# skhu101/TDNN-F_NAS

Measured on AMD Instinct MI355X. Metric: LF-MMI training frames/sec per node (SWBD 7q TDNN-F), higher is better.
Workload: dtype f32

## Files before the change

tdnn-f_nas_amd/csrc/abi_tdnn.hip:

```cpp
#include <dlfcn.h>
#include <stdlib.h>
#include <string.h>

#include <string>

#include "common.h"
#include "gemm_f32.h"
#include "planes_gemm.h"

namespace tdnnf {

static thread_local std::string g_last_error;

void set_error(const char *fmt, ...) {
  char buf[1024];
  va_list ap;
  va_start(ap, fmt);
  vsnprintf(buf, sizeof(buf), fmt, ap);
  va_end(ap);
  g_last_error = buf;
}
int hip_status(hipError_t e, const char *what) {
  set_error("HIP error %d (%s) in %s", (int)e, hipGetErrorString(e), what);
  return TDNNF_EHIP;
// ... 4 lines not shown
  return o;
}

namespace {
typedef int (*roctx_push_t)(const char *);
typedef int (*roctx_pop_t)();
roctx_push_t g_roctx_push = nullptr;
roctx_pop_t g_roctx_pop = nullptr;
bool roctx_ready() {
  static const bool ok = [] {
    const char *e = getenv("TDNNF_ROCTX");
    if (e && atoi(e) == 0) return false;
    for (const char *lib : {"librocprofiler-sdk-roctx.so", "librocprofiler-sdk-roctx.so.1", "libroctx64.so", "libroctx64.so.4"}) {
      void *h = dlopen(lib, RTLD_NOW | RTLD_GLOBAL);
      if (!h) continue;
      g_roctx_push = (roctx_push_t)dlsym(h, "roctxRangePushA");
      g_roctx_pop = (roctx_pop_t)dlsym(h, "roctxRangePop");
      if (g_roctx_push && g_roctx_pop) return true;
    }
    return false;
  }();
  return ok;
}
}
TraceRange::TraceRange(const char *name) : on(roctx_ready()) {
  if (on) g_roctx_push(name);
}
TraceRange::~TraceRange() {
  if (on) g_roctx_pop();
}

static bool tdnn_rows_ok(const tdnnf_tdnn_indexes *ix, int rows_in, int N) {
  if (!ix || ix->num_offsets < 1 || ix->num_offsets > TDNNF_MAX_OFFSETS || ix->row_stride < 1) return false;
  for (int i = 0; i < ix->num_offsets; i++) {
    const long long need = (long long)ix->row_offsets[i] + (long long)ix->row_stride * N - (ix->row_stride - 1);
    if (ix->row_offsets[i] < 0 || (N > 0 && rows_in < need)) return false;
  }
  return true;
}

}

using namespace tdnnf;

extern "C" {

const char *tdnnf_last_error(void) { return g_last_error.c_str(); }
int tdnnf_abi_version(void) { return 1; }

static int *option_slot(const char *name) {
  Options &o = options();
  if (!name) return nullptr;
  const struct { const char *n; int *p; } table[] = {{"ng_grouped", &o.ng_grouped}, {"ng_fuse", &o.ng_fuse}, {"ng_early_in", &o.ng_early_in},
                                                     {"wgrad_stream", &o.wgrad_stream}, {"gemm_ring", &o.gemm_ring}, {"planes", &o.planes}, {"den_split", &o.den_split}, {"phase_events", &o.phase_events}, {"wgrad_lag", &o.wgrad_lag}, {"ng_bk", &o.ng_bk}, {"ng_valu", &o.ng_valu}, {"ng_pform", &o.ng_pform}, {"planes_group", &o.planes_group}, {"xent_behind_den", &o.xent_behind_den}, {"ng_early_fork", &o.ng_early_fork}, {"ng_diag_skip", &o.ng_diag_skip}, {"wgrad_small", &o.wgrad_small}, {"splitk_per_cu", &o.splitk_per_cu}, {"gemm_alt_taps", &o.gemm_alt_taps}, {"reverse_passes", &o.reverse_passes}, {"splitk_partial_round", &o.splitk_partial_round}, {"wgrad_on_caller", &o.wgrad_on_caller}, {"den_mw_test_abort", &o.den_mw_test_abort}, {"planes_check_bound", &o.planes_check_bound}, {"den_gamma_pairs", &o.den_gamma_pairs}};
  for (auto &e : table)
    if (strcmp(e.n, name) == 0) return e.p;
  return nullptr;
}
int tdnnf_set_option(const char *name, int value) {
  int *p = option_slot(name);
  TDNNF_REQUIRE(p, "set_option: unknown option '%s' (ng_grouped, ng_fuse, ng_early_in, wgrad_stream, gemm_ring, planes, den_split)", name ? name : "(null)");
  *p = value;
  return TDNNF_OK;
}
int tdnnf_get_option(const char *name, int *value) {
  int *p = option_slot(name);
  TDNNF_REQUIRE(p && value, "get_option: unknown option '%s'", name ? name : "(null)");
  *value = *p;
  return TDNNF_OK;
}

}

namespace tdnnf {
int tdnn_propagate_impl(const tdnnf_tdnn_indexes *ix, const tdnnf_mat *in, const float *W, int ldw, int Do, int Di,
                        const float *bias, const float *eff_coef, int init_mode, int relu, tdnnf_mat *out, tdnnf_stream stream,
                        float *colstats, int *colstats_rows) {
  TDNNF_REQUIRE(mat_ok(in) && mat_ok(out) && W, "tdnn_propagate: bad matrices");
  TDNNF_REQUIRE(Do > 0 && Di > 0 && in->cols == Di && out->cols == Do, "tdnn_propagate: dims: in.cols=%d Di=%d out.cols=%d Do=%d",
                in ? in->cols : -1, Di, out ? out->cols : -1, Do);
  TDNNF_REQUIRE(tdnn_rows_ok(ix, in->rows, out->rows), "tdnn_propagate: input has too few rows for the time offsets");
  TDNNF_REQUIRE(ldw >= ix->num_offsets * Di, "tdnn_propagate: ldw < K*Di");
  TDNNF_REQUIRE(init_mode >= 0 && init_mode <= 2 && (init_mode != 1 || bias), "tdnn_propagate: init_mode 1 needs a bias");
  RowsGemmArgs a;
  memset(&a, 0, sizeof(a));
  a.A = in->data;
  a.lda = (long long)in->stride * ix->row_stride;
  a.B = W;
  a.ldb = ldw;
  a.C = out->data;
  a.ldc = out->stride;
  a.M = out->rows;
  a.N = Do;
  a.bias = bias;
  a.coef = eff_coef;
  a.init_mode = init_mode;
  a.relu = relu;
  a.colstats = colstats;
  a.colstats_rows = colstats_rows;
  a.nseg = ix->num_offsets;
  for (int i = 0; i < a.nseg; i++) {
    a.seg[i].a_off = (long long)ix->row_offsets[i] * in->stride;
    a.seg[i].b_off = (long long)i * Di;
    a.seg[i].klen = Di;
    a.seg[i].m_lo = 0;
    a.seg[i].m_hi = out->rows;
  }
// ... 201 lines not shown
```

tdnn-f_nas_amd/csrc/chain.hip:

```cpp
#include <math.h>
#include <string.h>

#include <algorithm>

#include <vector>

#include "common.h"
#include "gemm_f32.h"

struct tdnnf_den_graph {
  int H, A, P;
  struct Sell {
    int nrows, nslices;
    int *base;
    unsigned *row;
    uint2 *arc;
    uint4 *arc4;
    long long entries;
    int mw_max_arcs[9];
  } by_dst, by_src, by_pdf;
  float *init;
  float init_sum;
};

struct tdnnf_supervision {
  int B, T;
  int num_states, num_arcs;
  float weight;
  int *seq_state_begin;
  int *state_time;
  float *final_logprob;
  int *in_begin, *in_src, *in_pdf;
  float *in_lp;
  int *out_begin, *out_dst, *out_pdf;
  float *out_lp;
  int *frame_state_begin;
  int max_states_per_seq;
};

namespace tdnnf {
namespace {

constexpr int kDenThreads = 1024;
typedef float f32x4 __attribute__((ext_vector_type(4)));

__device__ __forceinline__ float block_sum(float v, float *red, int nwaves) {
  for (int o = 32; o > 0; o >>= 1) v += __shfl_xor(v, o, 64);
  __syncthreads();
  if ((threadIdx.x & 63) == 0) red[threadIdx.x >> 6] = v;
  __syncthreads();
  float s = 0.f;
  for (int w = 0; w < nwaves; w++) s += red[w];
  return s;
}

__device__ __forceinline__ float exp_limited(float v) {
  v = v < -30.f ? -30.f : (v > 30.f ? 30.f : v);
  return expf(v);
}

struct DenDev {
  int H, P;
  tdnnf_den_graph::Sell by_dst, by_src, by_pdf;
  const float *init;
  float init_sum;
};

constexpr int kDenRowRegs = 8;
struct RowAhead {
  float v[kDenRowRegs];
  __device__ __forceinline__ void load(const float *yr, int P, int tid) {
#pragma unroll
    for (int i = 0; i < kDenRowRegs; i++) {
      const int p = tid + i * kDenThreads;
      v[i] = p < P ? yr[p] : 0.f;
    }
  }
};

template <class Term>
__device__ __forceinline__ float sell_row_sum(const uint2 *ap, int w, Term term) {
  float acc = 0.f;
  int j = 0;
  for (; j + 8 <= w; j += 8) {
    uint2 a[8];
#pragma unroll
    for (int u = 0; u < 8; u++) a[u] = ap[(j + u) * 64];
#pragma unroll
    for (int u = 0; u < 8; u++) acc += term(a[u]);
  }
  if (j + 4 <= w) {
    uint2 a[4];
#pragma unroll
    for (int u = 0; u < 4; u++) a[u] = ap[(j + u) * 64];
#pragma unroll
    for (int u = 0; u < 4; u++) acc += term(a[u]);
    j += 4;
  }
  if (j < w) {
    uint2 a[3];
#pragma unroll
    for (int u = 0; u < 3; u++) a[u] = ap[min(j + u, w - 1) * 64];
#pragma unroll
    for (int u = 0; u < 3; u++) acc += (j + u < w) ? term(a[u]) : 0.f;
  }
  return acc;
}

constexpr int kDenFastSlots = 4, kDenFastStates = 4;
template <bool LDS_STATE, bool FAST = false>
__global__ __launch_bounds__(kDenThreads) void den_forward_kernel(DenDev g, MatView y, int B, int T, float leaky,
                                                                  float *alpha_all, float *asum_all, int Hs,
                                                                  double *logprob, float *gstate, const unsigned *only_if, int res_cap) {
  extern __shared__ __attribute__((aligned(16))) float smem[];
  __shared__ float red[kDenThreads / 64];
  if (only_if && *only_if == 0) return;
  const int s = blockIdx.x, tid = threadIdx.x;
  const int H = g.H, P = g.P;
  float *x = smem;
  float *prev = LDS_STATE ? smem + ((P + 3) & ~3) : gstate + (size_t)s * 2 * Hs;
  float *nxt = smem + ((P + 3) & ~3) + Hs;
  uint2 *lres = reinterpret_cast<uint2 *>(smem + ((P + 3) & ~3) + (LDS_STATE ? Hs : 0) + (FAST ? Hs : 0));
  for (int i = tid; i < res_cap; i += kDenThreads) lres[i] = g.by_dst.arc[i];
  int sb0[kDenFastSlots], sw[kDenFastSlots];
  unsigned srow[kDenFastSlots];
  float hinit[kDenFastStates];
// ... 589 lines not shown
  constexpr int kRows = 8;
  const int nslot = g.by_pdf.nslices * 64, ln = tid & 63;
  auto pa = [&](const uint2 a, int f) {
#pragma clang fp contract(off)
    return __uint_as_float(a.y) * smem[f * L + (a.x & 0xffffu)];
  };
  auto pb = [&](const uint2 a, int f) { return smem[f * L + H4 + (a.x >> 16)]; };
  for (int s0 = tid; s0 < nslot; s0 += kRows * kGamma2Threads) {
    int b0[kRows], w[kRows];
    unsigned row[kRows];
#pragma unroll
    for (int k = 0; k < kRows; k++) {
      const int slot = s0 + k * kGamma2Threads;
      b0[k] = 0;
      w[k] = 0;
      row[k] = 0xffffffffu;
      if (slot < nslot) {
        b0[k] = g.by_pdf.base[slot >> 6];
        w[k] = (g.by_pdf.base[(slot >> 6) + 1] - b0[k]) >> 6;
        row[k] = g.by_pdf.row[slot];
      }
    }
#pragma unroll
    for (int k = 0; k < kRows; k++) {
      if (row[k] == 0xffffffffu) continue;
      float acc[2];
      sell_row_sums<2>(g.by_pdf.arc + b0[k] + ln, w[k], acc, pa, pb);
#pragma unroll
      for (int f = 0; f < 2; f++) smem[f * L + 2 * H4 + row[k]] = scale[f] * acc[f];
    }
  }
  __syncthreads();
  constexpr int kOut = 6;
  for (int p0 = tid; p0 < P; p0 += kOut * kGamma2Threads) {
    float yv[2][kOut];
#pragma unroll
    for (int f = 0; f < 2; f++)
#pragma unroll
      for (int i = 0; i < kOut; i++) {
        const int p = p0 + i * kGamma2Threads;
        yv[f][i] = f < nf && p < P ? y.data[(size_t)((t0 + f) * B + s) * y.stride + p] : 0.f;
      }
#pragma unroll
    for (int f = 0; f < 2; f++) {
      if (f >= nf) break;
      const float *o = smem + f * L + 2 * H4;
      float *dr = deriv.data + (size_t)((t0 + f) * B + s) * deriv.stride;
#pragma unroll
      for (int i = 0; i < kOut; i++) {
        const int p = p0 + i * kGamma2Threads;
        if (p < P) dr[p] = o[p] * exp_limited(yv[f][i]);
      }
    }
  }
}
constexpr int kWideBatch = 8;
constexpr int kWideSlices = 2;

struct WideDims {
  int B, NG, SG;
};

typedef unsigned uv4 __attribute__((ext_vector_type(4)));

__global__ __launch_bounds__(256) void den_wide_prep_kernel(MatView y, WideDims d, int P, float *xT) {
  __shared__ float tile[64][65];
  const int t = blockIdx.z, p0 = blockIdx.x * 64, s0 = blockIdx.y * 64, tx = threadIdx.x & 63, ty = threadIdx.x >> 6;
  for (int i = ty; i < 64; i += 4) {
    const int sq = s0 + i, p = p0 + tx;
    tile[i][tx] = (sq < d.B && p < P) ? exp_limited(y.data[(size_t)(t * d.B + sq) * y.stride + p]) : 0.f;
  }
  __syncthreads();
  for (int i = ty; i < 64; i += 4) {
    const int p = p0 + i, sq = s0 + tx;
    if (p < P && sq < d.NG * d.SG) xT[(((size_t)t * d.NG + sq / d.SG) * P + p) * d.SG + sq % d.SG] = tile[tx][i];
  }
}
__global__ __launch_bounds__(256) void den_wide_unprep_kernel(const float *dT, WideDims d, int P, MatView deriv) {
  __shared__ float tile[64][65];
  const int t = blockIdx.z, p0 = blockIdx.x * 64, s0 = blockIdx.y * 64, tx = threadIdx.x & 63, ty = threadIdx.x >> 6;
  for (int i = ty; i < 64; i += 4) {
    const int p = p0 + i, sq = s0 + tx;
    tile[i][tx] = (p < P && sq < d.B) ? dT[(((size_t)t * d.NG + sq / d.SG) * P + p) * d.SG + sq % d.SG] : 0.f;
  }
  __syncthreads();
  for (int i = ty; i < 64; i += 4) {
    const int sq = s0 + i, p = p0 + tx;
    if (sq < d.B && p < P) deriv.data[(size_t)(t * d.B + sq) * deriv.stride + p] = tile[tx][i];
  }
}

__global__ __launch_bounds__(256) void den_wide_init_kernel(DenDev g, WideDims d, int Hs, bool ones, float *v, float *norm) {
  const long long total = (long long)d.NG * Hs * d.SG;
  for (long long e = blockIdx.x * 256LL + threadIdx.x; e < total; e += gridDim.x * 256LL) {
    const int h = (int)((e / d.SG) % Hs);
    v[e] = h < g.H ? (ones ? 1.0f : g.init[h]) : 0.f;
  }
  for (long long e = blockIdx.x * 256LL + threadIdx.x; e < d.B; e += gridDim.x * 256LL) norm[e] = g.init_sum;
}

template <int SG>
struct WideLane {
  static constexpr int RL = 64 / SG;
  static constexpr int IT = 16 / RL;
  int grp, blk, sl, rl, sq, wave, lane;
  bool on;
// ... 811 lines not shown
    TDNNF_HIP(hipStreamWaitEvent(aux, ev_fork, 0));
    int G = mw_groups(g, B, T);
    MwDev *md = mw_dev();
    if (!md) G = 0;
    if (G > 0 && !md->fallbacks) {
      if (hipHostMalloc((void **)&md->fallbacks, sizeof(unsigned), hipHostMallocMapped) != hipSuccess) {
        (void)hipGetLastError();
        md->fallbacks = nullptr;
        G = 0;
      } else {
        *md->fallbacks = 0;
      }
    }
    if (G > 0 && *(volatile unsigned *)md->fallbacks != 0) {
      fprintf(stderr, "tdnnf: the multi-workgroup denominator recursion timed out (its workgroups were not co-resident); the one-workgroup kernels redid the "
                      "minibatch and are used from here on (this device)\n");
      md->off = true;
      G = 0;
    }
    const size_t stage_b = G > 0 ? 256 * (size_t)((std::max(g->by_dst.nslices, g->by_src.nslices) + G - 1) / G) : 0;
    const size_t lds_f = G > 0 ? sizeof(float) * (P4 + H4) + 8 * (size_t)g->by_dst.mw_max_arcs[G] + stage_b : 0;
    const size_t lds_b = G > 0 ? sizeof(float) * (P4 + H4) + 8 * (size_t)g->by_src.mw_max_arcs[G] + stage_b : 0;
    if (G > 0) {
      TDNNF_HIP(hipFuncSetAttribute((const void *)den_mw_kernel<0>, hipFuncAttributeMaxDynamicSharedMemorySize, (int)lds_f));
      TDNNF_HIP(hipFuncSetAttribute((const void *)den_mw_kernel<1>, hipFuncAttributeMaxDynamicSharedMemorySize, (int)lds_b));
      int occ_f = 0, occ_b = 0;
      if (hipOccupancyMaxActiveBlocksPerMultiprocessor(&occ_f, den_mw_kernel<0>, kDenThreads, lds_f) != hipSuccess ||
          hipOccupancyMaxActiveBlocksPerMultiprocessor(&occ_b, den_mw_kernel<1>, kDenThreads, lds_b) != hipSuccess || occ_f < 1 || occ_b < 1 ||
          md->cus <= 0 || 2 * B * G > md->cus) {
        (void)hipGetLastError();
        G = 0;
      }
    }
    if (G > 0) {
      float *mw = S_all + (size_t)B * (T + 1) + 32;
      MwCtl ctl;
      ctl.NSp = (int)mw_slots(g);
      ctl.ctr = reinterpret_cast<unsigned long long *>((reinterpret_cast<uintptr_t>(mw) + 15) & ~(uintptr_t)15);
      ctl.abort_flag = reinterpret_cast<unsigned *>(ctl.ctr + 2 * B);
      ctl.xf = reinterpret_cast<float *>(ctl.ctr + 2 * B + 2);
      ctl.xb = ctl.xf + (size_t)B * 2 * ctl.NSp;
      TDNNF_HIP(hipMemsetAsync(ctl.ctr, 0, sizeof(unsigned long long) * (2 * B + 2), s));
      if (options().den_mw_test_abort) TDNNF_HIP(hipMemsetAsync(ctl.abort_flag, 1, 1, s));
      TDNNF_HIP(hipEventRecord(ev_fork, s));
      TDNNF_HIP(hipStreamWaitEvent(aux, ev_fork, 0));
      hipLaunchKernelGGL(den_mw_kernel<0>, dim3(B * G), dim3(kDenThreads), lds_f, s, gd, ctl, G, yv, B, T, leaky, b.alpha, b.asum, b.p.Hs, b.den_lp);
      hipLaunchKernelGGL(den_mw_kernel<1>, dim3(B * G), dim3(kDenThreads), lds_b, aux, gd, ctl, G, yv, B, T, leaky, b_all, S_all, b.p.Hs, (double *)nullptr);
      hipLaunchKernelGGL(den_forward_kernel<true>, dim3(B), dim3(kDenThreads), b.p.lds_fwd, s, gd, yv, B, T, leaky, b.alpha, b.asum, b.p.Hs, b.den_lp, b.gstate,
                         (const unsigned *)ctl.abort_flag, 0);
      hipLaunchKernelGGL(den_beta_kernel<false>, dim3(B), dim3(kDenThreads), lds_beta, aux, gd, yv, B, T, leaky, b_all, S_all, b.p.Hs, (const unsigned *)ctl.abort_flag, 0);
      hipLaunchKernelGGL(den_mw_check_kernel, dim3(1), dim3(64), 0, s, (const unsigned *)ctl.abort_flag, md->fallbacks);
    } else {
      const bool fast = g->by_dst.nslices * 64 <= kDenFastSlots * kDenThreads && g->by_src.nslices * 64 <= kDenFastSlots * kDenThreads && g->H <= kDenFastStates * kDenThreads;
      const size_t lf = b.p.lds_fwd + (fast ? sizeof(float) * b.p.Hs : 0), lb = lds_beta + (fast ? sizeof(float) * H4 : 0);
      int res_f = 0, res_b = 0;
      if (md && md->cus > 0 && 2 * B >= md->cus) {
        const size_t budget = 150 * 1024;
        if (lf < budget) res_f = (int)std::min<long long>(g->by_dst.entries, (long long)((budget - lf) / 8)) & ~63;
        if (lb < budget) res_b = (int)std::min<long long>(g->by_src.entries, (long long)((budget - lb) / 8)) & ~63;
      }
      (void)hipGetLastError();
      const size_t lds_f2 = lf + 8 * (size_t)res_f, lds_b2 = lb + 8 * (size_t)res_b;
      if (fast) {
        TDNNF_HIP(hipFuncSetAttribute((const void *)den_forward_kernel<true, true>, hipFuncAttributeMaxDynamicSharedMemorySize, (int)lds_f2));
        TDNNF_HIP(hipFuncSetAttribute((const void *)den_beta_kernel<true>, hipFuncAttributeMaxDynamicSharedMemorySize, (int)lds_b2));
        hipLaunchKernelGGL((den_forward_kernel<true, true>), dim3(B), dim3(kDenThreads), lds_f2, s, gd, yv, B, T, leaky, b.alpha, b.asum, b.p.Hs, b.den_lp, b.gstate,
                           (const unsigned *)nullptr, res_f);
        hipLaunchKernelGGL(den_beta_kernel<true>, dim3(B), dim3(kDenThreads), lds_b2, aux, gd, yv, B, T, leaky, b_all, S_all, b.p.Hs, (const unsigned *)nullptr, res_b);
      } else {
        TDNNF_HIP(hipFuncSetAttribute((const void *)den_forward_kernel<true>, hipFuncAttributeMaxDynamicSharedMemorySize, (int)lds_f2));
        TDNNF_HIP(hipFuncSetAttribute((const void *)den_beta_kernel<false>, hipFuncAttributeMaxDynamicSharedMemorySize, (int)lds_b2));
        hipLaunchKernelGGL(den_forward_kernel<true>, dim3(B), dim3(kDenThreads), lds_f2, s, gd, yv, B, T, leaky, b.alpha, b.asum, b.p.Hs, b.den_lp, b.gstate,
                           (const unsigned *)nullptr, res_f);
        hipLaunchKernelGGL(den_beta_kernel<false>, dim3(B), dim3(kDenThreads), lds_b2, aux, gd, yv, B, T, leaky, b_all, S_all, b.p.Hs, (const unsigned *)nullptr, res_b);
      }
    }
    TDNNF_HIP(hipEventRecord(ev_join, aux));
    TDNNF_HIP(hipStreamWaitEvent(s, ev_join, 0));
    if (ev_recursions) {
      TDNNF_HIP(hipEventRecord(ev_recursions, s));
      if (ev_recorded) *ev_recorded = true;
    }
    if (options().den_gamma_pairs != 1 && 2 * lds_gamma + sizeof(float) * kGamma2Threads / 64 <= kLdsBytes) {
      TDNNF_HIP(hipFuncSetAttribute((const void *)den_gamma2_kernel, hipFuncAttributeMaxDynamicSharedMemorySize, (int)(2 * lds_gamma)));
      hipLaunchKernelGGL(den_gamma2_kernel, dim3((T + 1) / 2, B), dim3(kGamma2Threads), 2 * lds_gamma, s, gd, yv, B, T, leaky, b.alpha, b_all, S_all, b.p.Hs, -sp->weight, dv);
    } else {
      TDNNF_HIP(hipFuncSetAttribute((const void *)den_gamma_kernel, hipFuncAttributeMaxDynamicSharedMemorySize, (int)lds_gamma));
      hipLaunchKernelGGL(den_gamma_kernel, dim3(T, B), dim3(kGammaThreads), lds_gamma, s, gd, yv, B, T, leaky, b.alpha, b_all, S_all, b.p.Hs, -sp->weight, dv);
    }
  } else if (b.p.lds_state) {
    TDNNF_HIP(hipFuncSetAttribute((const void *)den_backward_kernel<true>, hipFuncAttributeMaxDynamicSharedMemorySize, (int)b.p.lds_bwd));
    if (g->by_dst.nslices * 64 <= kDenFastSlots * kDenThreads && g->H <= kDenFastStates * kDenThreads) {
      const size_t lf = b.p.lds_fwd + sizeof(float) * b.p.Hs;
      TDNNF_HIP(hipFuncSetAttribute((const void *)den_forward_kernel<true, true>, hipFuncAttributeMaxDynamicSharedMemorySize, (int)lf));
      hipLaunchKernelGGL((den_forward_kernel<true, true>), dim3(B), dim3(kDenThreads), lf, s, gd, yv, B, T, leaky, b.alpha, b.asum, b.p.Hs, b.den_lp, b.gstate, (const unsigned *)nullptr, 0);
    } else {
      TDNNF_HIP(hipFuncSetAttribute((const void *)den_forward_kernel<true>, hipFuncAttributeMaxDynamicSharedMemorySize, (int)b.p.lds_fwd));
      hipLaunchKernelGGL(den_forward_kernel<true>, dim3(B), dim3(kDenThreads), b.p.lds_fwd, s, gd, yv, B, T, leaky, b.alpha, b.asum, b.p.Hs, b.den_lp, b.gstate, (const unsigned *)nullptr, 0);
    }
    hipLaunchKernelGGL(den_backward_kernel<true>, dim3(B), dim3(kDenThreads), b.p.lds_bwd, s, gd, yv, B, T, leaky, b.alpha, b.asum, b.p.Hs, -sp->weight, dv, b.gstate);
  } else {
    hipLaunchKernelGGL(den_forward_kernel<false>, dim3(B), dim3(kDenThreads), b.p.lds_fwd, s, gd, yv, B, T, leaky, b.alpha, b.asum, b.p.Hs, b.den_lp, b.gstate, (const unsigned *)nullptr, 0);
    hipLaunchKernelGGL(den_backward_kernel<false>, dim3(B), dim3(kDenThreads), b.p.lds_bwd, s, gd, yv, B, T, leaky, b.alpha, b.asum, b.p.Hs, -sp->weight, dv, b.gstate);
  }
  TDNNF_LAUNCH_CHECK();
  return TDNNF_OK;
}
float chain_supervision_weight(const tdnnf_supervision *sp) { return sp->weight; }
int chain_num_recursion(const tdnnf_supervision *sp, const tdnnf_den_graph *g, const tdnnf_mat *y, void *ws, hipStream_t s) {
  const int B = sp->B, T = sp->T;
  ChainBufs b = chain_bufs(g, B, T, ws);
  const MatView none{nullptr, 0, 0, 0};
  hipLaunchKernelGGL(numerator_kernel, dim3(B), dim3(64), 0, s, sup_dev(sp), view(y), none, b.la, b.lb, b.num_lp, b.xent, none, none, 0.f, 1);
  TDNNF_LAUNCH_CHECK();
  return TDNNF_OK;
}
// ... 65 lines not shown
```

tdnn-f_nas_amd/csrc/common.h:

```cpp
#pragma once
#include <hip/hip_runtime.h>
#include <stdarg.h>
#include <stdio.h>

#include "tdnnf_hip.h"

namespace tdnnf {

struct MatView {
  float *data;
  int rows, cols, stride;
};
inline MatView view(const tdnnf_mat *m) { return MatView{m->data, m->rows, m->cols, m->stride}; }

void set_error(const char *fmt, ...);
int hip_status(hipError_t e, const char *what);

inline bool mat_ok(const tdnnf_mat *m) {
  return m && m->rows >= 0 && m->cols >= 0 && m->stride >= m->cols && (m->data || m->rows * m->cols == 0);
}
inline bool same_dim(const tdnnf_mat *a, const tdnnf_mat *b) { return a->rows == b->rows && a->cols == b->cols; }

inline bool vec4_ok(const MatView &m) {
  return (reinterpret_cast<uintptr_t>(m.data) & 15) == 0 && m.stride % 4 == 0 && m.cols % 4 == 0;
}

#define TDNNF_REQUIRE(cond, ...)            \
  do {                                      \
    if (!(cond)) {                          \
      ::tdnnf::set_error(__VA_ARGS__);      \
      return TDNNF_EINVAL;                  \
    }                                       \
  } while (0)

#define TDNNF_HIP(expr)                                         \
  do {                                                          \
    hipError_t e__ = (expr);                                    \
    if (e__ != hipSuccess) return ::tdnnf::hip_status(e__, #expr); \
  } while (0)

#define TDNNF_LAUNCH_CHECK(name) TDNNF_HIP(hipGetLastError())

struct Options {
  int ng_grouped = 1;
  int ng_fuse = 1;
  int ng_early_in = 1;
  int wgrad_stream = -1;
  int gemm_ring = 1;
  int planes = 1;
  int den_mw_test_abort = 0;
  int planes_group = 1;
  int planes_check_bound = 0;
  int wgrad_lag = 3;
  int wgrad_on_caller = 0;
  int splitk_partial_round = 1;
  int reverse_passes = 0;
  int gemm_alt_taps = 1;
  int splitk_per_cu = 2;
  int wgrad_small = 0;
  int ng_bk = 0;
  int ng_early_fork = 1;
  int xent_behind_den = -1;
  int ng_pform = 1;
  int ng_valu = 0;
  int ng_diag_skip = 0;
  int phase_events = 0;
  int den_split = -1;
  int den_gamma_pairs = 0;
};
Options &options();

struct TraceRange {
  explicit TraceRange(const char *name);
  ~TraceRange();
  bool on;
};

__host__ __device__ inline float floor_keep_nan(float x, float f) { return x < f ? f : x; }

inline int grid_for(long long work, int block, int cap = 2048) {
  long long g = (work + block - 1) / block;
  if (g > cap) g = cap;
  if (g < 1) g = 1;
  return (int)g;
}

inline unsigned long long tdnnf_decision(unsigned long long step, unsigned long long k) {
  unsigned long long z = step * 0x9E3779B97F4A7C15ULL + k * 0xBF58476D1CE4E5B9ULL + 0x94D049BB133111EBULL;
  z = (z ^ (z >> 30)) * 0xBF58476D1CE4E5B9ULL;
  z = (z ^ (z >> 27)) * 0x94D049BB133111EBULL;
  return (z ^ (z >> 31)) >> 8;
}

constexpr int kFinCols = 8, kFinLanes = 32, kFinThreads = kFinCols * kFinLanes;
inline unsigned finalize_grid(int D) { return (unsigned)((D + kFinCols - 1) / kFinCols); }
#ifdef __HIPCC__
template <int NQ, class Acc>
__device__ __forceinline__ void finalize_sums(const float *partial, int chunks, long long qstride_rows, int D, int nq, Acc (&q)[NQ], Acc *red) {
  const int tc = threadIdx.x & (kFinCols - 1), lane = threadIdx.x / kFinCols, d = blockIdx.x * kFinCols + tc;
#pragma unroll
  for (int k = 0; k < NQ; k++) q[k] = 0;
  if (d < D) {
    const float *p = partial + d;
    const long long qs = qstride_rows * D;
    int c = lane;
    for (; c + 3 * kFinLanes < chunks; c += 4 * kFinLanes) {
      float v[NQ][4];
#pragma unroll
      for (int k = 0; k < NQ; k++) {
        if (k < nq) {
          const float *pk = p + (long long)k * qs;
          v[k][0] = pk[(long long)c * D]; v[k][1] = pk[(long long)(c + kFinLanes) * D];
          v[k][2] = pk[(long long)(c + 2 * kFinLanes) * D]; v[k][3] = pk[(long long)(c + 3 * kFinLanes) * D];
        }
      }
#pragma unroll
      for (int k = 0; k < NQ; k++) {
        if (k < nq) { q[k] += v[k][0]; q[k] += v[k][1]; q[k] += v[k][2]; q[k] += v[k][3]; }
      }
    }
    for (; c < chunks; c += kFinLanes) {
// ... 82 lines not shown
```

tdnn-f_nas_amd/csrc/net.hip:

```cpp
#include <math.h>
#include <string.h>

#include <functional>
#include <string>
#include <vector>

#include "common.h"
#include "fused.h"
#include "gemm_f32.h"
#include "gemm_ring.h"
#include "net.h"
#include "ng.h"
#include "optim_group.h"

namespace tdnnf {
namespace {

struct UpdTable {
  long long begin[129];
  float lr[128];
  float l2coef[128];
};

__global__ void add_scaled_taps_kernel(const float *G, const float *coef, float *acc, int Do, int KDi, int Di) {
// ... 1510 lines not shown
      CK(ng_stats_main(n->ng_in[comp], xin, n->ngc[comp].H_in, n->ngc[comp].part_in, n->ws4, n->ws_bytes, n->s4));
      E.done = n->fb_count;
    }
    if (forked) {
      TDNNF_HIP(hipEventRecord(n->ev_early, n->s4));
      n->early_any = true;
    }
    return TDNNF_OK;
  };
  const bool early_at_fork = n->early_on && !n->wg_on && !n->early_group && options().ng_early_fork != 0;
  if (early_at_fork) {
    CK(finish_refreshes());
    CK(launch_early_in(0));
  }
  const int No = n->Tout * B;
  tdnnf_mat top = M(prev, No, Hd), pl = M(n->prefinal_l_out, No, S);
  if (po_next.base == top.data && po_next.rows == top.rows) po_top = po_next;
  else CK(split(top, 0, kP | kT, &po_top, s, fb_next));
  {
    PlanesHintScope ph(hint_of(po_top), wplanes(n->c_prefinal_l));
    CK(tdnnf_affine_propagate(&top, Wp(n, n->c_prefinal_l), Hd, nullptr, S, &pl, s));
  }
  CK(split(pl, 0, kP | kT, &po_pl, s));
  tdnnf_mat y = M(n->head[0].y, No, P), dy = M(n->d_y, No, P), dx = M(n->d_xent, No, P);
  tdnnf_mat lsm = M(n->xent_logsoftmax, No, P);
  for (int h = 0; h < 2; h++) {
    auto &H = n->head[h];
    tdnnf_mat ar = M(H.aff_relu, No, Hd), lo = M(H.lin_out, No, S), b1 = M(H.bn1_out, No, Hd), b2 = M(H.bn2_out, No, S), yh = M(H.y, No, P);
    FroBound fb_b1;
    {
      PlanesHintScope ph(hint_of(po_pl), wplanes(H.c_affine));
      FroBoundScope fbs(pl_on ? n->fro_buf : nullptr, &fb_b1.blocks);
      CK(affine_relu_bn_stats(n, &ix1, &pl, Wp(n, H.c_affine), S, Hd, S, Bp(n, H.c_affine), nullptr, &ar, H.bn1_memo, H.bn1_stats, s));
    }
    CK(bn_apply_planes(ar, H.bn1_memo, none, 0.f, b1, nullptr, fb_b1, &po_b1[h]));
    if (!po_b1[h].base) CK(split(b1, 0, kP | kT, &po_b1[h], s, fb_b1));
    {
      PlanesHintScope ph(hint_of(po_b1[h]), wplanes(H.c_linear));
      CK(tdnnf_affine_propagate(&b1, Wp(n, H.c_linear), Hd, nullptr, S, &lo, s));
    }
    CK(bn_fwd(n, H.lin_out, H.bn2_out, No, S, H.bn2_memo, H.bn2_stats, s));
    CK(split(b2, 0, kP | kT, &po_b2[h], s));
    {
      PlanesHintScope ph(hint_of(po_b2[h]), wplanes(H.c_output));
      CK(tdnnf_affine_propagate(&b2, Wp(n, H.c_output), S, Bp(n, H.c_output), P, &yh, s));
    }
    if (h == 0) {
      TraceRange trace_den("chain denominator forward-backward (second stream)");
      TDNNF_HIP(hipEventRecord(n->ev_fork, s));
      TDNNF_HIP(hipStreamWaitEvent(n->s2, n->ev_fork, 0));
      const bool den_split = n->den_split;
      TDNNF_HIP(hipStreamWaitEvent(n->s3, n->ev_fork, 0));
      const int xbd = options().xent_behind_den;
      const bool behind = den_split && (xbd > 0 || (xbd < 0 && !n->wg_on));
      if (behind && !n->ev_den_rec) TDNNF_HIP(hipEventCreateWithFlags(&n->ev_den_rec, hipEventDisableTiming));
      bool rec = false;
      CK(chain_den(den, sup, &y, c.leaky_hmm, &dy, n->chain_ws, n->s2, !den_split, n->s3, behind ? n->ev_den_rec : nullptr, &rec));
      if (rec) TDNNF_HIP(hipStreamWaitEvent(s, n->ev_den_rec, 0));
      TDNNF_HIP(hipEventRecord(n->ev_den, n->s2));
      hipStream_t sn = n->s3;
      if (n->wg_on && den_split) {
        sn = n->s4;
        TDNNF_HIP(hipStreamWaitEvent(sn, n->ev_fork, 0));
      }
      CK(chain_num_recursion(sup, den, &y, n->chain_ws, sn));
      TDNNF_HIP(hipEventRecord(n->ev_num, sn));
    }
  }
  tdnnf_mat yx = M(n->head[1].y, No, P);
  const bool dense_first = log_softmax_propagate_with_aux(&yx, &lsm, &dx, -c.xent_regularize * chain_supervision_weight(sup), s);
  if (!dense_first) CK(tdnnf_log_softmax_propagate(&yx, &lsm, s));
  TDNNF_HIP(hipStreamWaitEvent(s, n->ev_num, 0));
  CK(chain_num_xent(den, sup, &y, &lsm, c.xent_regularize, &dx, n->chain_ws, s, dense_first));
  if (!dense_first) CK(tdnnf_log_softmax_backprop(&lsm, &dx, &dx, s));

  CK(phase_mark(n, 2, s));
  auto capture = [&](const std::string &name, const tdnnf_mat &m) -> int {
    if (!n->capture_on) return TDNNF_OK;
    tdnnf_mat *dst = nullptr;
    for (auto &kv : n->named)
      if (kv.first == name) dst = &kv.second;
    if (!dst) {
      float *p = nullptr;
      TDNNF_HIP(hipMalloc((void **)&p, sizeof(float) * (size_t)std::max(1, m.rows) * ldpad(m.cols)));
      n->captured.push_back(p);
      n->named.push_back({name, M(p, m.rows, m.cols)});
      dst = &n->named.back().second;
    }
    TDNNF_REQUIRE(dst->rows == m.rows && dst->cols == m.cols, "net_forward_backward: captured %s changed shape", name.c_str());
    return tdnnf_sum_scaled(&m, 1.0f, nullptr, 0.f, dst, s);
  };
  int fused_comp = -1;
  auto out_stats_fuse = [&](int comp, MatView xv, MatView dzv, MatView dv, NgFuse &f) -> int {
    fused_comp = -1;
    if (!c.use_natural_gradient || n->ng_out.empty() || !n->ng_out[comp] || n->comps[comp].lr_factor == 0.f) return 0;
    if (options().ng_fuse == 0) return 0;
    const bool fuse_always = options().ng_fuse == 2;
    auto &S = n->ngc[comp];
    const float *W = nullptr;
    int Rp = 0, ldw = 0;
    CK(ng_external_begin(n->ng_out[comp], dv.cols, &W, &Rp, &ldw, s));
    if (!W || !bn_relu_bwd_ng_ok(xv, dzv, dv, Rp) || !(fuse_always || bn_relu_bwd_ng_pays(dv.rows))) return 0;
    f.W = W; f.Rp = Rp; f.ldw = ldw; f.H = S.H_out; f.part = S.part_out; f.part_cap = rows_gemm_sumsq_blocks(dv.rows);
    fused_comp = comp;
    return 1;
  };
  unsigned long long relu_k = 0;
// ... 496 lines not shown
```

Before: 1.632 million.

## Process two sequences per block in denominator forward and backward kernels

```diff
diff --git a/tdnn-f_nas_amd/csrc/abi_tdnn.hip b/tdnn-f_nas_amd/csrc/abi_tdnn.hip
--- a/tdnn-f_nas_amd/csrc/abi_tdnn.hip
+++ b/tdnn-f_nas_amd/csrc/abi_tdnn.hip
@@ -80,7 +80,7 @@
   Options &o = options();
   if (!name) return nullptr;
   const struct { const char *n; int *p; } table[] = {{"ng_grouped", &o.ng_grouped}, {"ng_fuse", &o.ng_fuse}, {"ng_early_in", &o.ng_early_in},
-                                                     {"wgrad_stream", &o.wgrad_stream}, {"gemm_ring", &o.gemm_ring}, {"planes", &o.planes}, {"den_split", &o.den_split}, {"phase_events", &o.phase_events}, {"wgrad_lag", &o.wgrad_lag}, {"ng_bk", &o.ng_bk}, {"ng_valu", &o.ng_valu}, {"ng_pform", &o.ng_pform}, {"planes_group", &o.planes_group}, {"xent_behind_den", &o.xent_behind_den}, {"ng_early_fork", &o.ng_early_fork}, {"ng_diag_skip", &o.ng_diag_skip}, {"wgrad_small", &o.wgrad_small}, {"splitk_per_cu", &o.splitk_per_cu}, {"gemm_alt_taps", &o.gemm_alt_taps}, {"reverse_passes", &o.reverse_passes}, {"splitk_partial_round", &o.splitk_partial_round}, {"wgrad_on_caller", &o.wgrad_on_caller}, {"den_mw_test_abort", &o.den_mw_test_abort}, {"planes_check_bound", &o.planes_check_bound}, {"den_gamma_pairs", &o.den_gamma_pairs}};
+                                                     {"wgrad_stream", &o.wgrad_stream}, {"gemm_ring", &o.gemm_ring}, {"planes", &o.planes}, {"den_split", &o.den_split}, {"phase_events", &o.phase_events}, {"wgrad_lag", &o.wgrad_lag}, {"ng_bk", &o.ng_bk}, {"ng_valu", &o.ng_valu}, {"ng_pform", &o.ng_pform}, {"planes_group", &o.planes_group}, {"xent_behind_den", &o.xent_behind_den}, {"ng_early_fork", &o.ng_early_fork}, {"ng_diag_skip", &o.ng_diag_skip}, {"wgrad_small", &o.wgrad_small}, {"splitk_per_cu", &o.splitk_per_cu}, {"gemm_alt_taps", &o.gemm_alt_taps}, {"reverse_passes", &o.reverse_passes}, {"splitk_partial_round", &o.splitk_partial_round}, {"wgrad_on_caller", &o.wgrad_on_caller}, {"den_mw_test_abort", &o.den_mw_test_abort}, {"planes_check_bound", &o.planes_check_bound}, {"den_gamma_pairs", &o.den_gamma_pairs}, {"den_seq_pairs", &o.den_seq_pairs}};
   for (auto &e : table)
     if (strcmp(e.n, name) == 0) return e.p;
   return nullptr;
diff --git a/tdnn-f_nas_amd/csrc/chain.hip b/tdnn-f_nas_amd/csrc/chain.hip
--- a/tdnn-f_nas_amd/csrc/chain.hip
+++ b/tdnn-f_nas_amd/csrc/chain.hip
@@ -72,6 +72,18 @@
   __device__ __forceinline__ void load(const float *yr, int P, int tid) {
 #pragma unroll
     for (int i = 0; i < kDenRowRegs; i++) {
+      const int p = tid + i * kDenThreads;
+      v[i] = p < P ? yr[p] : 0.f;
+    }
+  }
+};
+
+constexpr int kDenRowRegs2 = 6;
+struct RowAhead2 {
+  float v[kDenRowRegs2];
+  __device__ __forceinline__ void load(const float *yr, int P, int tid) {
+#pragma unroll
+    for (int i = 0; i < kDenRowRegs2; i++) {
       const int p = tid + i * kDenThreads;
       v[i] = p < P ? yr[p] : 0.f;
     }
@@ -767,6 +779,274 @@
         if (p < P) dr[p] = o[p] * exp_limited(yv[f][i]);
       }
     }
+  }
+}
+
+__device__ __forceinline__ void block_sum2(float (&v)[2], float *red, int nwaves) {
+  for (int o = 32; o > 0; o >>= 1) {
+    v[0] += __shfl_xor(v[0], o, 64);
+    v[1] += __shfl_xor(v[1], o, 64);
+  }
+  __syncthreads();
+  if ((threadIdx.x & 63) == 0) {
+    red[threadIdx.x >> 6] = v[0];
+    red[nwaves + (threadIdx.x >> 6)] = v[1];
+  }
+  __syncthreads();
+  float s0 = 0.f, s1 = 0.f;
+  for (int w = 0; w < nwaves; w++) {
+    s0 += red[w];
+    s1 += red[nwaves + w];
+  }
+  v[0] = s0;
+  v[1] = s1;
+}
+
+__global__ __launch_bounds__(kDenThreads) void den_forward2_kernel(DenDev g, MatView y, int B, int T, float leaky, float *alpha_all, float *asum_all, int Hs,
+                                                                   double *logprob, int res_cap) {
+#pragma clang fp contract(off)
+  extern __shared__ __attribute__((aligned(16))) float smem[];
+  __shared__ float red[2 * kDenThreads / 64];
+  __shared__ double logcorr[2];
+  const int tid = threadIdx.x, s0 = 2 * blockIdx.x;
+  const bool two = s0 + 1 < B;
+  const int sq[2] = {s0, two ? s0 + 1 : s0};
+  const int H = g.H, P = g.P, P4 = (P + 3) & ~3;
+  float2 *x2 = reinterpret_cast<float2 *>(smem);
+  float2 *v2 = x2 + P4;
+  uint2 *lres = reinterpret_cast<uint2 *>(v2 + 2 * Hs);
+  for (int i = tid; i < res_cap; i += kDenThreads) lres[i] = g.by_dst.arc[i];
+  int sb0[kDenFastSlots], sw[kDenFastSlots];
+  unsigned srow[kDenFastSlots];
+  float hinit[kDenFastStates];
+#pragma unroll
+  for (int k = 0; k < kDenFastSlots; k++) {
+    const int slot = tid + k * kDenThreads;
+    sb0[k] = 0;
+    sw[k] = 0;
+    srow[k] = 0xffffffffu;
+    if (slot < g.by_dst.nslices * 64) {
+      sb0[k] = g.by_dst.base[slot >> 6];
+      sw[k] = (g.by_dst.base[(slot >> 6) + 1] - sb0[k]) >> 6;
+      srow[k] = g.by_dst.row[slot];
+    }
+  }
+#pragma unroll
+  for (int i = 0; i < kDenFastStates; i++) hinit[i] = tid + i * kDenThreads < H ? g.init[tid + i * kDenThreads] : 0.f;
+  float *alpha[2], *asum[2];
+#pragma unroll
+  for (int n = 0; n < 2; n++) {
+    alpha[n] = alpha_all + (size_t)sq[n] * (T + 1) * Hs;
+    asum[n] = asum_all + (size_t)sq[n] * (T + 1);
+  }
+
+  for (int h = tid; h < H; h += kDenThreads) {
+    const float a = __builtin_fmaf(leaky * g.init_sum, g.init[h], g.init[h]);
+    v2[h] = make_float2(a, a);
+    alpha[0][h] = a;
+    if (two) alpha[1][h] = a;
+  }
+  if (tid == 0) {
+    asum[0][0] = g.init_sum;
+    if (two) asum[1][0] = g.init_sum;
+  }
+  float prev_sum[2] = {g.init_sum, g.init_sum};
+  if (tid == 0) logcorr[0] = logcorr[1] = 0.0;
+  int cp = 0;
+  RowAhead2 ra[2];
+#pragma unroll
+  for (int n = 0; n < 2; n++) ra[n].load(y.data + (size_t)sq[n] * y.stride, P, tid);
+  __syncthreads();
+  for (int t = 1; t <= T; t++) {
+#pragma unroll
+    for (int i = 0; i < kDenRowRegs2; i++)
+      if (tid + i * kDenThreads < P) x2[tid + i * kDenThreads] = make_float2(exp_limited(ra[0].v[i]), exp_limited(ra[1].v[i]));
+    for (int p = tid + kDenRowRegs2 * kDenThreads; p < P; p += kDenThreads)
+      x2[p] = make_float2(exp_limited(y.data[(size_t)((t - 1) * B + sq[0]) * y.stride + p]), exp_limited(y.data[(size_t)((t - 1) * B + sq[1]) * y.stride + p]));
+    if (t < T) {
+#pragma unroll
+      for (int n = 0; n < 2; n++) ra[n].load(y.data + (size_t)(t * B + sq[n]) * y.stride, P, tid);
+    }
+    __syncthreads();
+    float inv[2];
+#pragma unroll
+    for (int n = 0; n < 2; n++) {
+      inv[n] = 1.0f / prev_sum[n];
+      if (tid == 0) logcorr[n] += (double)logf(prev_sum[n]);
+    }
+    const float2 *prv = v2 + cp * Hs;
+    float2 *nx = v2 + (1 - cp) * Hs;
+    auto pa = [&](const uint2 a, int n) {
+      const float2 v = prv[a.x & 0xffffu];
+      return (n ? v.y : v.x) * __uint_as_float(a.y);
+    };
+    auto pb = [&](const uint2 a, int n) {
+      const float2 v = x2[a.x >> 16];
+      return n ? v.y : v.x;
+    };
+    float local[2] = {0.f, 0.f};
+    const int ln = tid & 63;
+#pragma unroll
+    for (int k = 0; k < kDenFastSlots; k++) {
+      if (srow[k] == 0xffffffffu && sw[k] == 0) continue;
+      float acc[2];
+      int b0 = sb0[k];
+      asm volatile("" : "+v"(b0));
+      if (b0 + sw[k] * 64 <= res_cap)
+        sell_row_sums<2>(lres + b0 + ln, sw[k], acc, pa, pb);
+      else
+        sell_row_sums<2>(g.by_dst.arc + b0 + ln, sw[k], acc, pa, pb);
+      if (srow[k] != 0xffffffffu) {
+        nx[srow[k]] = make_float2(acc[0] * inv[0], acc[1] * inv[1]);
+#pragma unroll
+        for (int n = 0; n < 2; n++) local[n] = __builtin_fmaf(acc[n], inv[n], local[n]);
+      }
+    }
+    block_sum2(local, red, kDenThreads / 64);
+    if (tid == 0) {
+      asum[0][t] = local[0];
+      if (two) asum[1][t] = local[1];
+    }
+#pragma unroll
+    for (int i = 0; i < kDenFastStates; i++) {
+      const int h = tid + i * kDenThreads;
+      if (h < H) {
+        const float2 v = nx[h];
+        const float a0 = __builtin_fmaf(leaky * local[0], hinit[i], v.x), a1 = __builtin_fmaf(leaky * local[1], hinit[i], v.y);
+        nx[h] = make_float2(a0, a1);
+        alpha[0][(size_t)t * Hs + h] = a0;
+        if (two) alpha[1][(size_t)t * Hs + h] = a1;
+      }
+    }
+    cp ^= 1;
+    prev_sum[0] = local[0];
+    prev_sum[1] = local[1];
+    __syncthreads();
+  }
+  float local[2] = {0.f, 0.f};
+  for (int h = tid; h < H; h += kDenThreads) {
+    const float2 v = v2[cp * Hs + h];
+    local[0] += v.x;
+    local[1] += v.y;
+  }
+  block_sum2(local, red, kDenThreads / 64);
+  if (tid == 0) {
+#pragma unroll
+    for (int n = 0; n < 2; n++) {
+      if (n == 1 && !two) break;
+      logprob[sq[n]] = (double)logf(local[n]) + logcorr[n];
+      asum[n][T] = local[n];
+    }
+  }
+}
+
+__global__ __launch_bounds__(kDenThreads) void den_beta2_kernel(DenDev g, MatView y, int B, int T, float leaky, float *b_all, float *S_all, int Hs, int res_cap) {
+#pragma clang fp contract(off)
+  extern __shared__ __attribute__((aligned(16))) float smem[];
+  __shared__ float red[2 * kDenThreads / 64];
+  const int tid = threadIdx.x, s0 = 2 * blockIdx.x;
+  const bool two = s0 + 1 < B;
+  const int sq[2] = {s0, two ? s0 + 1 : s0};
+  const int H = g.H, P = g.P, P4 = (P + 3) & ~3, H4 = (H + 3) & ~3;
+  float2 *x2 = reinterpret_cast<float2 *>(smem);
+  float2 *bn = x2 + P4;
+  float2 *nb = bn + H4;
+  uint2 *lres = reinterpret_cast<uint2 *>(nb + H4);
+  for (int i = tid; i < res_cap; i += kDenThreads) lres[i] = g.by_src.arc[i];
+  int sb0[kDenFastSlots], sw[kDenFastSlots];
+  unsigned srow[kDenFastSlots];
+  float sinit[kDenFastSlots];
+#pragma unroll
+  for (int k = 0; k < kDenFastSlots; k++) {
+    const int slot = tid + k * kDenThreads;
+    sb0[k] = 0;
+    sw[k] = 0;
+    srow[k] = 0xffffffffu;
+    sinit[k] = 0.f;
+    if (slot < g.by_src.nslices * 64) {
+      sb0[k] = g.by_src.base[slot >> 6];
+      sw[k] = (g.by_src.base[(slot >> 6) + 1] - sb0[k]) >> 6;
+      srow[k] = g.by_src.row[slot];
+      if (srow[k] != 0xffffffffu) sinit[k] = g.init[srow[k]];
+    }
+  }
+  float *brow[2], *S[2];
+#pragma unroll
+  for (int n = 0; n < 2; n++) {
+    brow[n] = b_all + (size_t)sq[n] * (T + 1) * Hs;
+    S[n] = S_all + (size_t)sq[n] * (T + 1);
+  }
+  for (int h = tid; h < H; h += kDenThreads) {
+    const float v = 1.0f / g.init_sum + leaky;
+    brow[0][(size_t)T * Hs + h] = 1.0f;
+    if (two) brow[1][(size_t)T * Hs + h] = 1.0f;
+    bn[h] = make_float2(v, v);
+  }
+  if (tid == 0) {
+    S[0][T] = g.init_sum;
+    if (two) S[1][T] = g.init_sum;
+  }
+  RowAhead2 ra[2];
+#pragma unroll
+  for (int n = 0; n < 2; n++) ra[n].load(y.data + (size_t)((T - 1) * B + sq[n]) * y.stride, P, tid);
+  __syncthreads();
+  for (int t = T - 1; t >= 0; t--) {
+#pragma unroll
+    for (int i = 0; i < kDenRowRegs2; i++)
+      if (tid + i * kDenThreads < P) x2[tid + i * kDenThreads] = make_float2(exp_limited(ra[0].v[i]), exp_limited(ra[1].v[i]));
+    for (int p = tid + kDenRowRegs2 * kDenThreads; p < P; p += kDenThreads)
+      x2[p] = make_float2(exp_limited(y.data[(size_t)(t * B + sq[0]) * y.stride + p]), exp_limited(y.data[(size_t)(t * B + sq[1]) * y.stride + p]));
+    if (t > 0) {
+#pragma unroll
+      for (int n = 0; n < 2; n++) ra[n].load(y.data + (size_t)((t - 1) * B + sq[n]) * y.stride, P, tid);
+    }
+    __syncthreads();
+    auto pa = [&](const uint2 a, int n) {
+      const float2 v = x2[a.x >> 16];
+      return __uint_as_float(a.y) * (n ? v.y : v.x);
+    };
+    auto pb = [&](const uint2 a, int n) {
+      const float2 v = bn[a.x & 0xffffu];
+      return n ? v.y : v.x;
+    };
+    float local[2] = {0.f, 0.f};
+    const int ln = tid & 63;
+#pragma unroll
+    for (int k = 0; k < kDenFastSlots; k++) {
+      if (srow[k] == 0xffffffffu && sw[k] == 0) continue;
+      float acc[2];
+      int b0 = sb0[k];
+      asm volatile("" : "+v"(b0));
+      if (b0 + sw[k] * 64 <= res_cap)
+        sell_row_sums<2>(lres + b0 + ln, sw[k], acc, pa, pb);
+      else
+        sell_row_sums<2>(g.by_src.arc + b0 + ln, sw[k], acc, pa, pb);
+      if (srow[k] != 0xffffffffu) {
+        nb[srow[k]] = make_float2(acc[0], acc[1]);
+#pragma unroll
+        for (int n = 0; n < 2; n++) local[n] = __builtin_fmaf(sinit[k], acc[n], local[n]);
+      }
+    }
+    block_sum2(local, red, kDenThreads / 64);
+    if (tid == 0) {
+      S[0][t] = local[0];
+      if (two) S[1][t] = local[1];
+    }
+    float inv[2];
+#pragma unroll
+    for (int n = 0; n < 2; n++) inv[n] = 1.0f / local[n];
+#pragma unroll
+    for (int i = 0; i < kDenFastStates; i++) {
+      int h = tid + i * kDenThreads;
+      asm volatile("" : "+v"(h));
+      if (h < H) {
+        const float2 v = nb[h];
+        brow[0][(size_t)t * Hs + h] = v.x;
+        if (two) brow[1][(size_t)t * Hs + h] = v.y;
+        bn[h] = make_float2(__builtin_fmaf(v.x, inv[0], leaky), __builtin_fmaf(v.y, inv[1], leaky));
+      }
+    }
+    __syncthreads();
   }
 }
 constexpr int kWideBatch = 8;
@@ -1684,7 +1964,9 @@
       hipLaunchKernelGGL(den_mw_check_kernel, dim3(1), dim3(64), 0, s, (const unsigned *)ctl.abort_flag, md->fallbacks);
     } else {
       const bool fast = g->by_dst.nslices * 64 <= kDenFastSlots * kDenThreads && g->by_src.nslices * 64 <= kDenFastSlots * kDenThreads && g->H <= kDenFastStates * kDenThreads;
-      const size_t lf = b.p.lds_fwd + (fast ? sizeof(float) * b.p.Hs : 0), lb = lds_beta + (fast ? sizeof(float) * H4 : 0);
+      const size_t lf0 = b.p.lds_fwd + (fast ? sizeof(float) * b.p.Hs : 0), lb0 = lds_beta + (fast ? sizeof(float) * H4 : 0);
+      const bool pairs = fast && options().den_seq_pairs != 1 && 2 * std::max(lf0, lb0) + sizeof(float) * 2 * kDenThreads / 64 <= kLdsBytes;
+      const size_t lf = pairs ? 2 * lf0 : lf0, lb = pairs ? 2 * lb0 : lb0;
       int res_f = 0, res_b = 0;
       if (md && md->cus > 0 && 2 * B >= md->cus) {
         const size_t budget = 150 * 1024;
@@ -1693,7 +1975,12 @@
       }
       (void)hipGetLastError();
       const size_t lds_f2 = lf + 8 * (size_t)res_f, lds_b2 = lb + 8 * (size_t)res_b;
-      if (fast) {
+      if (pairs) {
+        TDNNF_HIP(hipFuncSetAttribute((const void *)den_forward2_kernel, hipFuncAttributeMaxDynamicSharedMemorySize, (int)lds_f2));
+        TDNNF_HIP(hipFuncSetAttribute((const void *)den_beta2_kernel, hipFuncAttributeMaxDynamicSharedMemorySize, (int)lds_b2));
+        hipLaunchKernelGGL(den_forward2_kernel, dim3((B + 1) / 2), dim3(kDenThreads), lds_f2, s, gd, yv, B, T, leaky, b.alpha, b.asum, b.p.Hs, b.den_lp, res_f);
+        hipLaunchKernelGGL(den_beta2_kernel, dim3((B + 1) / 2), dim3(kDenThreads), lds_b2, aux, gd, yv, B, T, leaky, b_all, S_all, b.p.Hs, res_b);
+      } else if (fast) {
         TDNNF_HIP(hipFuncSetAttribute((const void *)den_forward_kernel<true, true>, hipFuncAttributeMaxDynamicSharedMemorySize, (int)lds_f2));
         TDNNF_HIP(hipFuncSetAttribute((const void *)den_beta_kernel<true>, hipFuncAttributeMaxDynamicSharedMemorySize, (int)lds_b2));
         hipLaunchKernelGGL((den_forward_kernel<true, true>), dim3(B), dim3(kDenThreads), lds_f2, s, gd, yv, B, T, leaky, b.alpha, b.asum, b.p.Hs, b.den_lp, b.gstate,
diff --git a/tdnn-f_nas_amd/csrc/common.h b/tdnn-f_nas_amd/csrc/common.h
--- a/tdnn-f_nas_amd/csrc/common.h
+++ b/tdnn-f_nas_amd/csrc/common.h
@@ -67,6 +67,7 @@
   int phase_events = 0;
   int den_split = -1;
   int den_gamma_pairs = 0;
+  int den_seq_pairs = 0;
 };
 Options &options();
 
diff --git a/tdnn-f_nas_amd/csrc/net.hip b/tdnn-f_nas_amd/csrc/net.hip
--- a/tdnn-f_nas_amd/csrc/net.hip
+++ b/tdnn-f_nas_amd/csrc/net.hip
@@ -1586,7 +1586,7 @@
       const bool den_split = n->den_split;
       TDNNF_HIP(hipStreamWaitEvent(n->s3, n->ev_fork, 0));
       const int xbd = options().xent_behind_den;
-      const bool behind = den_split && (xbd > 0 || (xbd < 0 && !n->wg_on));
+      const bool behind = den_split && (xbd > 0 || (xbd < 0 && !n->wg_on && options().den_seq_pairs == 1));
       if (behind && !n->ev_den_rec) TDNNF_HIP(hipEventCreateWithFlags(&n->ev_den_rec, hipEventDisableTiming));
       bool rec = false;
       CK(chain_den(den, sup, &y, c.leaky_hmm, &dy, n->chain_ws, n->s2, !den_split, n->s3, behind ? n->ev_den_rec : nullptr, &rec));
```

Result: faster. 1.649 million (median of 6 runs) (+1.0%).
